# goofoo/SLR

Hardware: AMD Instinct MI355X
Metric: Msamples/sec @1024spp 1280x720 (unidirectional path tracing, Cornell_Box_Spheres-shaped scene) (higher is better)
Workload: dtype f32; 1 GPU; BASELINE configs[1]: Cornell_Box_Spheres walls/light/camera (TestScenes/Cornell_Box_Spheres.txt:8-107,132-138) + two tessellated spheres (aluminium mirror, Lambert), 4428 triangles, RGB mode, 1280x720, 1024 spp, seed 1509761209; stripes=0, tree=host binned SAH

## Files before the change

### slr_amd/csrc/pt_kernels.h

```cpp
#pragma once
#include <hip/hip_runtime.h>
#include <stdint.h>

#include "device_types.h"

namespace slrhip {

static const int kLdsMaterials = 32;
static const int kLdsLights = 16;
static const int kLdsSpectra = 96;
static const int kLdsPoolFloats = 6144;

struct DevScene {
    const float4* nodes;
    const float4* leafTris;
    const ShadeTri* shadeTris;
    const LightTri* lightTris;
    const DevMaterial* materials;
    const DevMaterialS* materialsS;
    const DevSpectrum* spectra;
    const float* spectrumPool;
    const float* lightPMF;
    const float* lightCDF;
    uint32_t numNodes;
// ... 51 lines not shown

struct PathBuffers {
    uint4* rng;
    float4* rayOrg;
    float4* rayDir;
    float4* hit;
    int32_t* hitInstance;
    float4* alpha;
    float4* spR;
    float4* spC;
    float4* results;
    float4* fbSum;
    float4* fbComp;
    float4* nee;
    float4* shadowDir;
    float* pdfPrev;
    uint4* hdr;
    uint32_t* flags;
    uint32_t* cursor;
    uint32_t* visible;
    uint32_t* shadowQueue;
    uint32_t* tailList;
    uint32_t* queueCount;
    uint32_t* activeSlots;
    uint32_t* idleShards;
    uint32_t* blockDead;
    uint32_t* errorWord;
    uint32_t* tailMode;
    uint32_t* tailWords;
    uint32_t* tailIdled;
    uint32_t* windowSamples;
    uint64_t* totals;
    const uint32_t* pixelXY;
    uint32_t rayStride, spStride, hdrStride;
};

struct RenderParams {
    uint32_t numSlots;
    uint32_t numBlocks;
    uint32_t numPixels, stripes;
    uint32_t sppBegin, sppCount;
    uint32_t workItems;
    uint32_t numWaves;
    uint32_t runLength;
    uint32_t numRuns;
    int32_t rngSeed;
    float timeStart, timeEnd;
    uint32_t imageWidth, imageHeight;
    uint32_t countSlots;
    uint32_t shardCapacity;
    uint32_t spectral;
    uint32_t injectError;
    uint32_t tailSlots;
};

static const uint32_t kWorkRotate = 40503u;
struct WorkItem {
    uint32_t pix, pass;
    bool valid;
};
__host__ __device__ inline uint32_t workRun(const RenderParams& rp, uint32_t wave, uint32_t j) {
    return j * rp.numWaves + (uint32_t)(((uint64_t)wave + (uint64_t)j * kWorkRotate) % rp.numWaves);
}
__host__ __device__ inline WorkItem workItemOf(const RenderParams& rp, uint32_t wave, uint32_t taken) {
    const uint32_t j = taken / rp.runLength, r = taken - j * rp.runLength;
    WorkItem w;
    w.pix = 0; w.pass = 0; w.valid = false;
    if (j > rp.numRuns / rp.numWaves) return w;
    const uint32_t run = workRun(rp, wave, j);
    if (run >= rp.numRuns) return w;
    const uint32_t group = run / rp.numPixels;
    w.pix = run - group * rp.numPixels;
    w.pass = group * rp.runLength + r;
    w.valid = true;
    return w;
}
__host__ __device__ inline uint32_t workSamplesTaken(const RenderParams& rp, uint32_t wave, uint32_t taken) {
    uint32_t runs = 0;
    for (uint32_t j = 0; j <= rp.numRuns / rp.numWaves; ++j) if (workRun(rp, wave, j) < rp.numRuns) ++runs;
    const uint32_t length = runs * rp.runLength;
    return taken < length ? taken : length;
}

__device__ __forceinline__ uint32_t liveSlots(const PathBuffers& pb, uint32_t numSlots) {
    uint32_t idle = 0;
#pragma unroll
    for (uint32_t k = 0; k < kShards; ++k) idle += pb.idleShards[k * kCounterStride];
    return numSlots - idle;
}
__device__ __forceinline__ bool tailModeBegins(const PathBuffers& pb, uint32_t live, uint32_t tailSlots, uint32_t parity) {
    if (tailSlots == 0u) return false;
    if (pb.tailMode[0]) return true;
    if (live > tailSlots) return false;
    if (blockIdx.x == 0 && threadIdx.x == 0) pb.tailMode[0] = 1u + parity;
    return true;
}

void launchResetSlots(const PathBuffers& pb, const RenderParams& rp, bool clearSensor, hipStream_t stream);
void launchFold(const PathBuffers& pb, const RenderParams& rp, hipStream_t stream);
void launchShade(const DevScene& sc, const PathBuffers& pb, const RenderParams& rp, uint32_t parity, hipStream_t stream);
void launchCountSamples(const PathBuffers& pb, const RenderParams& rp, hipStream_t stream);
void launchTail(const DevScene& sc, const PathBuffers& pb, const RenderParams& rp, uint32_t liveSlots, int numCUs, hipStream_t stream);
bool tailKernelAvailable(const DevScene& sc, bool spectral);
void launchResolve(const PathBuffers& pb, const RenderParams& rp, float* dst, hipStream_t stream);
void launchBsdfQueries(const DevScene& sc, bool spectral, uint32_t material, uint32_t n, const float* in, float wlOffset, uint32_t wl,
                       float4* geo, float4* misc, float4* fsSample, float4* fsEval, hipStream_t stream);
// ... 30 lines not shown
```

### slr_amd/csrc/pt_shade_kernels.h

```cpp
#pragma once
#include <hip/hip_runtime.h>
#include <stdlib.h>

#include <string>

#include "pt_bsdf.h"
#include "pt_bsdf_multi.h"
#include "pt_camera.h"
#include "pt_kernels.h"
#include "pt_surface.h"
#include "pt_tex.h"

namespace slrhip {

enum : uint32_t {
    ST_IDLE = 0,
    ST_REGEN = 1,
    ST_FIRST_HIT = 2,
    ST_NEXT_HIT = 3,
    ST_FINISH = 4
};
#define F_STATE(f) ((f) & 7u)
#define F_PATHLEN(f) (((f) >> 3) & 127u)
#define F_WL(f) (((f) >> 16) & 15u)
#define F_WLSEL(f) (((f) >> 12) & 1u)
#define F_DELTA(f) (((f) >> 13) & 1u)
#define F_SHADOW(f) (((f) >> 14) & 1u)
#define F_HASPATH(f) (((f) >> 15) & 1u)
#define F_SPVALID(f) (((f) >> 10) & 1u)
#define F_MAKE(state, len, wl, wlsel, delta, shadow) \
    ((state) | ((len) << 3) | ((wl) << 16) | ((wlsel) << 12) | ((delta) << 13) | ((shadow) << 14))

static const int kShadeBlock = 256;

template <class S> struct SpecIO;
template <> struct SpecIO<RGB> {
    static __device__ __forceinline__ void load(const float4* a, const float* , uint32_t slot, uint32_t , RGB& v, float& w) {
        const float4 q = a[slot];
        v = RGB(q.x, q.y, q.z); w = q.w;
    }
    static __device__ __forceinline__ void store(float4* a, float* , uint32_t slot, uint32_t , const RGB& v, float w) {
        a[slot] = make_float4(v.r, v.g, v.b, w);
    }
};
template <> struct SpecIO<Spec16> {
    static __device__ __forceinline__ void load(const float4* a, const float* scalars, uint32_t slot, uint32_t n, Spec16& v, float& w) {
#pragma unroll
        for (int p = 0; p < 4; ++p) {
            const float4 q = a[(size_t)p * n + slot];
            v.c[4 * p] = q.x; v.c[4 * p + 1] = q.y; v.c[4 * p + 2] = q.z; v.c[4 * p + 3] = q.w;
        }
        w = scalars ? scalars[slot] : 0.0f;
    }
    static __device__ __forceinline__ void store(float4* a, float* scalars, uint32_t slot, uint32_t n, const Spec16& v, float w) {
#pragma unroll
        for (int p = 0; p < 4; ++p) a[(size_t)p * n + slot] = make_float4(v.c[4 * p], v.c[4 * p + 1], v.c[4 * p + 2], v.c[4 * p + 3]);
        if (scalars) scalars[slot] = w;
    }
};

template <class S> struct MatIO;
template <> struct MatIO<RGB> {
    template <bool LDS>
    static __device__ __forceinline__ Mat<RGB> load(const DevScene& sc, const float4* ldsMats, uint32_t idx, float) {
// ... 251 lines not shown
    __device__ __forceinline__ void end(const PathBuffers&, uint32_t, uint32_t, bool) {}
};

template <bool SPECTRAL>
struct ShadeLds {
    float4 mats[SPECTRAL ? kLdsMaterials * 2 + kLdsSpectra * 2 + kLdsPoolFloats / 4 : kLdsMaterials * 5];
    float4 lights[kLdsLights * 9];
    float lightPMF[kLdsLights];
    float lightCDF[kLdsLights + 4];
};
static_assert(kLdsLights % 4 == 0, "the light PMF is staged as whole float4");

template <bool SPECTRAL>
__device__ __forceinline__ void stageShadeTables(const DevScene& sc, ShadeLds<SPECTRAL>& lds) {
    constexpr uint32_t kSegments = SPECTRAL ? 6u : 4u;
    constexpr uint32_t matsF4 = SPECTRAL ? kLdsMaterials * 2 + kLdsSpectra * 2 + kLdsPoolFloats / 4 : kLdsMaterials * 5;
    const uint32_t dst[6] = {0u,
                             SPECTRAL ? (uint32_t)(kLdsMaterials * 2) : matsF4,
                             SPECTRAL ? (uint32_t)(kLdsMaterials * 2 + kLdsSpectra * 2) : matsF4 + kLdsLights * 9,
                             SPECTRAL ? matsF4 : matsF4 + kLdsLights * 9 + kLdsLights / 4,
                             matsF4 + kLdsLights * 9,
                             matsF4 + kLdsLights * 9 + kLdsLights / 4};
    float4* out = reinterpret_cast<float4*>(&lds);
    const uint32_t total = sc.tableEnd[kSegments - 1];
    for (uint32_t base = threadIdx.x; base < total; base += 4 * kShadeBlock) {
        float4 v[4];
#pragma unroll
        for (int u = 0; u < 4; ++u) {
            const uint32_t i = base + u * kShadeBlock;
            v[u] = sc.shadeTables[min(i, total - 1u)];
        }
#pragma unroll
        for (int u = 0; u < 4; ++u) asm volatile("" : "+v"(v[u].x), "+v"(v[u].y), "+v"(v[u].z), "+v"(v[u].w));
#pragma unroll
        for (int u = 0; u < 4; ++u) {
            const uint32_t i = base + u * kShadeBlock;
            if (i >= total) continue;
            uint32_t begin = 0, to = dst[0];
#pragma unroll
            for (uint32_t k = 0; k + 1 < kSegments; ++k)
                if (i >= sc.tableEnd[k]) { begin = sc.tableEnd[k]; to = dst[k + 1]; }
            out[to + (i - begin)] = v[u];
        }
    }
}

#ifndef SLR_WAVES_SPECTRAL_GLOSSY
#define SLR_WAVES_SPECTRAL_GLOSSY 2
#endif
#ifndef SLR_WAVES_SPECTRAL
#define SLR_WAVES_SPECTRAL 3
#endif
#ifndef SLR_WAVES_RGB
#define SLR_WAVES_RGB 2
#endif
template <class S> struct TexSpectrum {
    static __device__ __forceinline__ S eval(const DevScene& sc, const DevTexture& t, float texU, float texV, float wlOffset) {
        if (t.kind == SLRHIP_TEXTURE_IMAGE_SPECTRUM) {
            const float* x = sc.texTexels + (size_t)imageTexel(t, texU, texV) * 3;
            const float kEqualEnergyReflectance = 0.009355121400914532f;
            return evaluateUpsampledRuntime<S>(sc, x[0], x[1], x[2] / kEqualEnergyReflectance, wlOffset);
        }
        return evalSpectrum<S>(sc.spectra, sc.spectrumPool, checkerIndex(t, texU, texV) ? t.spec1 : t.spec0, wlOffset);
    }
};
template <> struct TexSpectrum<RGB> {
    static __device__ __forceinline__ RGB eval(const DevScene& sc, const DevTexture& t, float texU, float texV, float) {
        if (t.kind == SLRHIP_TEXTURE_IMAGE_SPECTRUM) {
            const float* x = sc.texTexels + (size_t)imageTexel(t, texU, texV) * 3;
            return RGB(x[0], x[1], x[2]);
        }
        return checkerIndex(t, texU, texV) ? RGB(t.rgb1[0], t.rgb1[1], t.rgb1[2]) : RGB(t.rgb0[0], t.rgb0[1], t.rgb0[2]);
    }
};

template <class S>
__device__ __forceinline__ int32_t texturizeMat(const DevScene& sc, Mat<S>& mm, uint32_t matIndex, float texU, float texV, float wlOffset) {
    mm.type &= ~kMatTexturedBit;
    const int4 mt = *reinterpret_cast<const int4*>(sc.matTex + matIndex);
    if (mt.x >= 0) { const DevTexture t = loadTexture(sc.textures, (uint32_t)mt.x); mm.a = 1.0f * TexSpectrum<S>::eval(sc, t, texU, texV, wlOffset); }
    if (mt.y >= 0) { const DevTexture t = loadTexture(sc.textures, (uint32_t)mt.y); mm.b = TexSpectrum<S>::eval(sc, t, texU, texV, wlOffset); }
    if (mt.z >= 0) { const DevTexture t = loadTexture(sc.textures, (uint32_t)mt.z); mm.c = TexSpectrum<S>::eval(sc, t, texU, texV, wlOffset); }
    return mt.w;
}

template <class S>
struct SlotLoads {
    uint4 r4;
    S alpha;
    float pdfPrev;
    float4 h, o4, d4;
    int32_t hitInstance;
    float wlOffset;
    __device__ __forceinline__ void issue(const DevScene& sc, const PathBuffers& pb, const RenderParams& rp, uint32_t slot) {
        r4 = pb.rng[(size_t)slot * pb.hdrStride];
        SpecIO<S>::load(pb.alpha, pb.pdfPrev, slot, rp.numSlots, alpha, pdfPrev);
        h = pb.hit[slot];
        hitInstance = sc.instances ? pb.hitInstance[slot] : -1;
        o4 = pb.rayOrg[(size_t)slot * pb.rayStride];
        d4 = pb.rayDir[(size_t)slot * pb.rayStride];
        wlOffset = S::N == 3 ? 0.0f : __uint_as_float(pb.hdr[(size_t)slot * pb.hdrStride].z);
    }
};

template <class S, bool LDS_TABLES, bool MF, bool MULTI, bool TEX, bool FUSED>
__device__ __forceinline__ void logicSlot(const DevScene& sc, const PathBuffers& pb, const RenderParams& rp, const ShadeLds<S::N != 3>& lds,
                                          const float* lightPMF, const float* lightCDF, uint32_t slot, const SlotLoads<S>& in, uint32_t& flags, uint32_t vis,
// ... 265 lines not shown

        flags |= sp.validBits();
        if (FUSED && emitRegen) {
            radiance = sp.total();
        }
        else {
            pb.flags[slot] = flags;
            sp.end(pb, slot, rp.numSlots, !emitRegen);
        }
        if (!emitRegen) {
            pb.rng[(size_t)slot * pb.hdrStride] = make_uint4(rng.s0, rng.s1, rng.s2, rng.s3);
            SpecIO<S>::store(pb.alpha, pb.pdfPrev, slot, rp.numSlots, alpha, bsdfPDFprev);
        }
        if (emitExt) {
            pb.rayOrg[(size_t)slot * pb.rayStride] = make_float4(rayOrg.x, rayOrg.y, rayOrg.z, rayTmin);
            pb.rayDir[(size_t)slot * pb.rayStride] = make_float4(rayDir.x, rayDir.y, rayDir.z, INFINITY);
        }
    }
}

__device__ __forceinline__ RGB storageAddend(const RGB& val, float) { return val; }
__device__ __forceinline__ Spec16 storageAddend(const Spec16& val, float wlOffset) {
    const float recBinWidth = 16 / (830.0f - 360.0f);
    uint32_t sBin[16];
    float v[16];
    bool near = true;
#pragma unroll
    for (int i = 0; i < 16; ++i) {
        sBin[i] = min((uint32_t)((wavelengthOf(i, wlOffset) - 360.0f) / (830.0f - 360.0f) * 16), 15u);
        v[i] = val.c[i] * recBinWidth;
        near = near && (sBin[i] + 1u >= (uint32_t)i) && (sBin[i] <= (uint32_t)i + 1u);
    }
    Spec16 addend;
    if (near) {
#pragma unroll
        for (int b = 0; b < 16; ++b) {
            float a = 0.0f;
            if (b > 0) a = (sBin[b - 1] == (uint32_t)b) ? a + v[b - 1] : a;
            a = (sBin[b] == (uint32_t)b) ? a + v[b] : a;
            if (b < 15) a = (sBin[b + 1] == (uint32_t)b) ? a + v[b + 1] : a;
            addend.c[b] = a;
        }
    }
    else {
#pragma unroll
        for (int i = 0; i < 16; ++i) {
#pragma unroll
            for (int b = 0; b < 16; ++b) addend.c[b] = (sBin[i] == (uint32_t)b) ? addend.c[b] + v[i] : addend.c[b];
        }
    }
    return addend;
}

template <class S>
__device__ __forceinline__ void startSample(const DevScene& sc, const PathBuffers& pb, const RenderParams& rp, uint32_t slot, uint32_t pix,
                                            uint32_t passOfWindow) {
    const uint32_t xy = pb.pixelXY[pix];
    const uint32_t px = xy & 0xFFFFu, py = xy >> 16;
    Rng rng;
    const CameraDraws draws = drawCameraSample(rng, rp.rngSeed, px, py, rp.sppBegin + passOfWindow, rp.timeStart, rp.timeEnd);
    const float wlOffset = draws.wlOffset;
    const uint32_t wl = min((uint32_t)(uint16_t)(S::N * draws.uLambda), (uint32_t)(S::N - 1));
    const float selectWLPDF = S::N == 3 ? 1.0f : S::N / (830.0f - 360.0f);
    const CameraRay cam = sampleCameraRay(sc.camera, rp.imageWidth, rp.imageHeight, draws);
    const V3 lensP = cam.org, lensN = cam.lensN, rayDir = cam.dir;
    float dirPDF = sc.camera.imgPlaneDistance * sc.camera.imgPlaneDistance /
                   ((cam.dirLocalZ * cam.dirLocalZ * cam.dirLocalZ) * sc.camera.imgPlaneArea);
    float camWeight = absDot(rayDir, lensN) / (sc.camera.areaPDF * dirPDF * selectWLPDF);
    pb.flags[slot] = F_MAKE((uint32_t)ST_FIRST_HIT, 0u, wl, 0u, 0u, 0u);
    pb.rng[(size_t)slot * pb.hdrStride] = make_uint4(rng.s0, rng.s1, rng.s2, rng.s3);
    pb.hdr[(size_t)slot * pb.hdrStride] = make_uint4(pix, __float_as_uint(camWeight), __float_as_uint(wlOffset), passOfWindow);
    pb.rayOrg[(size_t)slot * pb.rayStride] = make_float4(lensP.x, lensP.y, lensP.z, 0.0f);
    pb.rayDir[(size_t)slot * pb.rayStride] = make_float4(rayDir.x, rayDir.y, rayDir.z, INFINITY);
}

__device__ __forceinline__ void storeResult(float4* results, size_t entry, const RGB& v) { results[entry] = make_float4(v.r, v.g, v.b, 0.0f); }
__device__ __forceinline__ void storeResult(float4* results, size_t entry, const Spec16& v) {
#pragma unroll
    for (int k = 0; k < 4; ++k) results[entry * 4 + k] = make_float4(v.c[4 * k], v.c[4 * k + 1], v.c[4 * k + 2], v.c[4 * k + 3]);
}
template <class S>
__device__ __forceinline__ void writeResult(const PathBuffers& pb, const RenderParams& rp, uint32_t slot, uint32_t flags, const uint4& hdr,
                                            bool inRegisters, S C) {
    float unusedW;
    const float camW = __uint_as_float(hdr.y);
    if (!inRegisters) {
        C = S();
        if (F_SPVALID(flags)) SpecIO<S>::load(pb.spR, nullptr, slot * pb.spStride, rp.numSlots * pb.spStride, C, unusedW);
    }
    const S weight = (S(1.0f) * S(1.0f)) * camW;
    storeResult(pb.results, (size_t)hdr.w * rp.numPixels + hdr.x, storageAddend(weight * C, S::N == 3 ? 0.0f : __uint_as_float(hdr.z)));
}

struct StartLds {
    uint32_t lane[kShadeBlock];
    uint32_t pix[kShadeBlock];
    uint32_t pass[kShadeBlock];
    uint32_t waveBase[kShadeBlock / 64 + 1];
    uint32_t wentIdle;
};

#ifndef SLR_SHADE_EARLY
#define SLR_SHADE_EARLY 1
#endif
template <class S, bool LDS_TABLES, bool MF, bool MULTI = false, bool TEX = false>
__global__ __launch_bounds__(kShadeBlock)
__attribute__((amdgpu_waves_per_eu(S::N == 3 ? SLR_WAVES_RGB : (MF ? SLR_WAVES_SPECTRAL_GLOSSY : SLR_WAVES_SPECTRAL)))) void k_shade(DevScene sc, PathBuffers pb, RenderParams rp, uint32_t parity) {
    __shared__ ShadeLds<S::N != 3> lds;
    __shared__ PushLds pushLds;
    __shared__ StartLds start;
    const uint32_t slot = blockIdx.x * kShadeBlock + threadIdx.x;
    const uint32_t lane = threadIdx.x & 63u, wave = threadIdx.x >> 6;

    {
        const uint32_t liveSlots = pb.activeSlots[0], tailMode = pb.tailMode[0], dead = pb.blockDead[blockIdx.x];
        if ((liveSlots == 0u) | (tailMode != 0u) | (dead != 0u)) return;
    }

    uint32_t flags = pb.flags[slot];
    const uint32_t vis = pb.visible[slot];
    SlotLoads<S> in;
    if (SLR_SHADE_EARLY) in.issue(sc, pb, rp, slot);
    const uint32_t state0 = F_STATE(flags);
    const uint32_t globalWave = blockIdx.x * (kShadeBlock / 64) + wave;
    const uint32_t taken = pb.cursor[globalWave];
    if (threadIdx.x == 0) start.wentIdle = 0u;
    if (LDS_TABLES) stageShadeTables<S::N != 3>(sc, lds);
    {
        const int anyWork = __syncthreads_or(state0 != ST_IDLE);
        if (!anyWork) {
            if (threadIdx.x == 0) pb.blockDead[blockIdx.x] = 1u;
            return;
        }
    }
    if (!SLR_SHADE_EARLY) in.issue(sc, pb, rp, slot);
    const float* lightPMF = LDS_TABLES ? lds.lightPMF : sc.lightPMF;
    const float* lightCDF = LDS_TABLES ? lds.lightCDF : sc.lightCDF;

    bool emitExt = false, emitShadow = false, pathEnded = false;
    S radiance;
    if (state0 == ST_FIRST_HIT || state0 == ST_NEXT_HIT || state0 == ST_FINISH)
        logicSlot<S, LDS_TABLES, MF, MULTI, TEX, true>(sc, pb, rp, lds, lightPMF, lightCDF, slot, in, flags, vis, radiance, emitExt, emitShadow, pathEnded);

    if (pathEnded) {
        const uint4 hdr = pb.hdr[(size_t)slot * pb.hdrStride];
        writeResult<S>(pb, rp, slot, flags, hdr, S::N == 3, radiance);
    }
    blockPush(pushLds, emitShadow, slot, pb.shadowQueue, pb.queueCount + parity * kQueueSetWords, rp.shardCapacity, pb.errorWord);
    if (rp.countSlots) {
        const uint64_t ma = __ballot(emitExt || emitShadow || pathEnded);
        if (lane == 0 && ma) atomicAdd((unsigned long long*)&pb.totals[totalIndex(T_SLOT_VISITS, blockIdx.x % kShards)], (unsigned long long)__popcll(ma));
    }

    const bool wants = pathEnded || state0 == ST_REGEN;
    {
        const uint64_t mw = __ballot(wants);
        WorkItem w;
        w.valid = false;
        if (wants) w = workItemOf(rp, globalWave, taken + (uint32_t)__popcll(mw & ((1ull << lane) - 1ull)));
        if (lane == 0 && mw) pb.cursor[globalWave] = taken + (uint32_t)__popcll(mw);
        const bool becameIdle = wants && !w.valid;
        if (becameIdle) pb.flags[slot] = F_MAKE((uint32_t)ST_IDLE, 0u, 0u, 0u, 0u, 0u);
        const uint64_t mi = __ballot(becameIdle);
        if (lane == 0 && mi) atomicAdd(&start.wentIdle, (uint32_t)__popcll(mi));
        const bool starts = wants && w.valid;
        const uint64_t ms = __ballot(starts);
        if (lane == 0) start.waveBase[wave] = (uint32_t)__popcll(ms);
        __syncthreads();
        uint32_t base = 0;
        for (uint32_t k = 0; k < wave; ++k) base += start.waveBase[k];
        if (starts) {
            const uint32_t i = base + (uint32_t)__popcll(ms & ((1ull << lane) - 1ull));
            start.lane[i] = threadIdx.x;
            start.pix[i] = w.pix;
            start.pass[i] = w.pass;
        }
        __syncthreads();
        if (threadIdx.x == 0 && start.wentIdle) atomicAdd(&pb.idleShards[(blockIdx.x % kShards) * kCounterStride], start.wentIdle);
        const uint32_t n = start.waveBase[0] + start.waveBase[1] + start.waveBase[2] + start.waveBase[3];
        if (threadIdx.x < n)
            startSample<S>(sc, pb, rp, blockIdx.x * kShadeBlock + start.lane[threadIdx.x], start.pix[threadIdx.x], start.pass[threadIdx.x]);
    }
}

template <class S>
__global__ void k_reset_slots(PathBuffers pb, RenderParams rp, uint32_t clearSensor) {
    const uint32_t slot = blockIdx.x * blockDim.x + threadIdx.x;
    pb.flags[slot] = F_MAKE((uint32_t)ST_REGEN, 0u, 0u, 0u, 0u, 0u);
    pb.hdr[(size_t)slot * pb.hdrStride] = make_uint4(0u, 0u, 0u, 0u);
    pb.visible[slot] = 0;
    if (threadIdx.x == 0) pb.blockDead[blockIdx.x] = 0u;
    if ((threadIdx.x & 63u) == 0u) pb.cursor[slot >> 6] = 0u;
    if (clearSensor) {
        constexpr uint32_t planes = S::N == 3 ? 1u : 4u;
        for (size_t e = slot; e < (size_t)rp.numPixels * planes; e += (size_t)gridDim.x * blockDim.x) {
            pb.fbSum[e] = make_float4(0.0f, 0.0f, 0.0f, 0.0f);
            pb.fbComp[e] = make_float4(0.0f, 0.0f, 0.0f, 0.0f);
        }
    }
    if (blockIdx.x == 0) {
        for (uint32_t k = threadIdx.x; k < 2 * kQueueSetWords; k += blockDim.x) pb.queueCount[k] = 0;
        if (threadIdx.x < kShards) pb.idleShards[threadIdx.x * kCounterStride] = 0u;
        if (threadIdx.x == 0) {
            pb.activeSlots[0] = rp.numSlots; pb.errorWord[0] = rp.injectError ? ERR_QUEUE_OVERFLOW : 0u;
            pb.tailMode[0] = 0u; pb.tailWords[0] = 0u; pb.tailWords[1] = 0u; pb.tailIdled[0] = 0u; pb.windowSamples[0] = 0u;
        }
    }
}

template <class S>
__global__ void k_resolve(PathBuffers pb, RenderParams rp, float* dst) {
    const uint32_t pix = blockIdx.x * blockDim.x + threadIdx.x;
    if (pix >= rp.numPixels) return;
    const uint32_t xy = pb.pixelXY[pix];
    const uint32_t px = xy & 0xFFFFu, py = xy >> 16;
    float* o = dst + ((size_t)py * rp.imageWidth + px) * S::N;
    if (S::N == 3) {
        const float4 v = pb.fbSum[pix];
        o[0] = v.x; o[1] = v.y; o[2] = v.z;
    }
    else {
#pragma unroll
        for (int k = 0; k < 4; ++k) {
            const float4 v = pb.fbSum[(size_t)pix * 4 + k];
            o[4 * k] = v.x; o[4 * k + 1] = v.y; o[4 * k + 2] = v.z; o[4 * k + 3] = v.w;
        }
    }
}

template <class S>
__global__ void __launch_bounds__(64) k_bsdf_queries(DevScene sc, uint32_t material, uint32_t n, const float* __restrict__ in, float wlOffset,
                                                     uint32_t wl, float4* __restrict__ geo, float4* __restrict__ misc,
                                                     float4* __restrict__ fsSample, float4* __restrict__ fsEval) {
    const uint32_t i = blockIdx.x * blockDim.x + threadIdx.x;
// ... 38 lines not shown
```

### slr_amd/csrc/slrhip_api.hip

```cpp
#include <hip/hip_runtime.h>
#include <dlfcn.h>

#include <algorithm>
#include <atomic>
#include <chrono>
#include <cmath>
#include <cstdio>
#include <cstring>
#include <string>
#include <vector>

#include "../../include/slrhip.h"
#include "bvh.h"
#include "pt_kernels.h"
#include "render_plan.h"
#include "scene_prep.h"

using namespace slrhip;

namespace {

const int kDefaultPairs = 1;
const uint32_t kStatusWords = 8;
enum StatusWord : uint32_t {
// ... 212 lines not shown
        if (const int rc = checkTreeLimits(g.depth, g.numNodes, g.numLeafTris,
                                           "device-built tree deeper than the 64-entry traversal stack (QBVH.h:299); use the host build", &err)) {
            for (void* a : {(void*)g.nodes, (void*)g.nodesQ, (void*)g.leafTris, (void*)g.shadeTris}) (void)hipFree(a);
            return fail(rc, err);
        }
        ctx->nodes.adopt(g.nodes, g.numNodes);
        ctx->leafTris.adopt(g.leafTris, g.numLeafTris);
        ctx->shadeTris.adopt(g.shadeTris, d.num_triangles);
        quantized = g.nodesQ != nullptr && useQuantizedNodes(g.numNodes);
        if (quantized) ctx->nodesQ.adopt(g.nodesQ, g.numNodes); else (void)hipFree(g.nodesQ);
        numNodes = g.numNodes; depth = g.depth; leafRefs = g.numLeafTris;
    }
    else {
        HIP_TRY(ctx->nodes.upload(p.bvh.nodes));
        if (p.quantized) HIP_TRY(ctx->nodesQ.upload(p.bvh.quantized));
        if (p.wide8) HIP_TRY(ctx->nodes8.upload(p.bvh.nodes8));
        HIP_TRY(ctx->leafTris.upload(p.bvh.leafTris));
    }
    HIP_TRY(ctx->textures.upload(p.textures));
    HIP_TRY(ctx->texTexels.upload(p.texTexels));
    HIP_TRY(ctx->matTex.upload(p.matTex));
    HIP_TRY(ctx->triUV.upload(p.triUV));
    HIP_TRY(ctx->alphaTris.upload(p.alphaTris));
    if (p.build != TreeBuild::Device) HIP_TRY(ctx->shadeTris.upload(p.shadeTris));
    HIP_TRY(ctx->lightTris.upload(p.lightTris));
    HIP_TRY(ctx->instances.upload(p.instances));
    HIP_TRY(ctx->materials.upload(p.materials));
    HIP_TRY(ctx->materialsS.upload(p.materialsS));
    HIP_TRY(ctx->spectrumPool.upload(p.spectrumPool));
    HIP_TRY(ctx->spectra.upload(p.spectra));
    HIP_TRY(ctx->lightPMF.upload(p.lightPMF));
    HIP_TRY(ctx->lightCDF.upload(p.lightCDF));
    HIP_TRY(ctx->shadeTables.upload(p.shadeTables));
    HIP_TRY(ctx->envTexels.upload(p.envTexels));
    HIP_TRY(ctx->envTopPDF.upload(p.envTopPDF)); HIP_TRY(ctx->envTopCDF.upload(p.envTopCDF));
    HIP_TRY(ctx->envRowPDF.upload(p.envRowPDF)); HIP_TRY(ctx->envRowCDF.upload(p.envRowCDF));
    HIP_TRY(ctx->gridCells.upload(p.gridCells)); HIP_TRY(ctx->pointUV.upload(p.pointUV)); HIP_TRY(ctx->pointSpectrum.upload(p.pointSpectrum));
    HIP_TRY(ctx->queryError.alloc(1));
    HIP_TRY(hipMemset(ctx->queryError.ptr, 0, sizeof(uint32_t)));
    bindScene(ctx, d, p, numNodes, quantized);
    ctx->bvhDepth = depth;
    ctx->bvhLeafRefs = leafRefs;
    ctx->haveScene = true;
    return SLRHIP_OK;
}

static long autoStripesOverride() { static const long v = [] { const char* e = tuningEnv("SLRHIP_AUTO_STRIPES"); return e ? atol(e) : 0L; }(); return v; }
static int pairsMask() { static const int v = [] { const char* e = tuningEnv("SLRHIP_PAIRS"); return e ? atoi(e) : kDefaultPairs; }(); return v; }
static uint32_t runLengthOverride() {
    static const uint32_t v = [] { const char* e = getenv("SLRHIP_RUN_LENGTH"); const long n = e ? atol(e) : 0L; return n >= 1 && n <= 4096 ? (uint32_t)n : 0u; }();
    return v;
}

static size_t frameFloats(const RenderParams& rp) { return (size_t)rp.imageWidth * rp.imageHeight * (rp.spectral ? 16 : 3); }

static void bindBuffers(slrhip_ctx* ctx, const FramePlan& plan) {
    PathBuffers pb{};
    pb.rayStride = plan.rayStride; pb.spStride = plan.spStride; pb.hdrStride = plan.hdrStride;
    pb.rayOrg = ctx->rayOrg.ptr; pb.rayDir = plan.rayStride == 2 ? ctx->rayOrg.ptr + 1 : ctx->rayDir.ptr;
    pb.spR = ctx->spR.ptr; pb.spC = plan.spStride == 2 ? ctx->spR.ptr + 1 : ctx->spC.ptr;
    pb.hdr = ctx->hdr.ptr; pb.rng = plan.hdrStride == 2 ? ctx->hdr.ptr + 1 : ctx->rng.ptr;
    pb.hit = ctx->hit.ptr; pb.hitInstance = ctx->scene.instances ? ctx->hitInstance.ptr : nullptr;
    pb.alpha = ctx->alpha.ptr; pb.pdfPrev = plan.spectral ? ctx->pdfPrev.ptr : nullptr;
    pb.nee = ctx->nee.ptr; pb.shadowDir = ctx->shadowDir.ptr; pb.visible = ctx->visible.ptr; pb.flags = ctx->flags.ptr;
    pb.results = ctx->results.ptr; pb.fbSum = ctx->fbSum.ptr; pb.fbComp = ctx->fbComp.ptr; pb.pixelXY = ctx->pixelXY.ptr;
    pb.cursor = ctx->cursor.ptr; pb.shadowQueue = ctx->shadowQueue.ptr; pb.tailList = ctx->tailList.ptr; pb.queueCount = ctx->queueCount.ptr;
    pb.idleShards = ctx->idleShards.ptr; pb.blockDead = ctx->blockDead.ptr; pb.totals = ctx->totals.ptr;
    uint32_t* const status = ctx->activeSlots.ptr;
    pb.activeSlots = status + S_LIVE; pb.errorWord = status + S_ERROR; pb.windowSamples = status + S_WINDOW_SAMPLES;
    pb.tailIdled = status + S_TAIL_IDLED; pb.tailMode = status + S_TAIL_MODE; pb.tailWords = status + S_TAIL_LENGTH;
    ctx->buffers = pb;
}

static hipError_t readStatus(slrhip_ctx* ctx, uint32_t* words, uint32_t count, hipStream_t s) {
    const hipError_t e = hipMemcpyAsync(words, ctx->activeSlots.ptr, count * sizeof(uint32_t), hipMemcpyDeviceToHost, s);
    return e == hipSuccess ? hipStreamSynchronize(s) : e;
}

static int checkWindow(slrhip_ctx* ctx, hipStream_t s) {
    uint32_t words[kStatusWords] = {};
    HIP_TRY(readStatus(ctx, words, kStatusWords, s));
    if (words[S_ERROR]) return deviceError(words[S_ERROR]);
    if (words[S_WINDOW_SAMPLES] != ctx->params.workItems)
        return fail(SLRHIP_ERR_HIP, "slrhip_render: the work queues handed out " + std::to_string(words[S_WINDOW_SAMPLES]) + " samples for a window of " +
                                        std::to_string(ctx->params.workItems) + " (internal error)");
    return SLRHIP_OK;
}

static int runTail(slrhip_ctx* ctx, uint32_t* status, hipStream_t s, bool timed) {
    struct Timer {
        hipEvent_t t0 = nullptr, t1 = nullptr;
        ~Timer() { if (t0) (void)hipEventDestroy(t0); if (t1) (void)hipEventDestroy(t1); }
    } timer;
    if (timed) { HIP_TRY(hipEventCreate(&timer.t0)); HIP_TRY(hipEventCreate(&timer.t1)); HIP_TRY(hipEventRecord(timer.t0, s)); }
    launchTail(ctx->scene, ctx->buffers, ctx->params, status[S_LIVE], ctx->numCUs, s);
    if (timed) HIP_TRY(hipEventRecord(timer.t1, s));
    HIP_TRY(hipGetLastError());
    const uint32_t liveBefore = status[S_LIVE];
    uint32_t words[S_TAIL_CURSOR + 1] = {};
    HIP_TRY(readStatus(ctx, words, S_TAIL_CURSOR + 1, s));
    std::memcpy(status, words, (S_TAIL_MODE + 1) * sizeof(uint32_t));
    if (timed) {
        float ms = 0.0f;
        HIP_TRY(hipEventElapsedTime(&ms, timer.t0, timer.t1));
        ctx->profMs[SLRHIP_KERNEL_TAIL] += ms;
        ++ctx->profLaunches[SLRHIP_KERNEL_TAIL];
// ... 166 lines not shown

int slrhip_upload_scene(slrhip_ctx* ctx, const slrhip_scene_desc* d) {
    if (!ctx || !d) return fail(SLRHIP_ERR_INVALID_ARGUMENT, "slrhip_upload_scene: null argument");
    const auto t0 = std::chrono::steady_clock::now();
    PreparedScene p;
    std::string err;
    if (const int rc = prepareScene(*d, ctx->config, &p, &err)) return fail(rc, err);
    if (const int rc = commitScene(ctx, *d, p)) return rc;
    ctx->buildSeconds = std::chrono::duration<double>(std::chrono::steady_clock::now() - t0).count();
    return SLRHIP_OK;
}

int slrhip_render_begin(slrhip_ctx* ctx, const slrhip_render_settings* st, slrhip_shard shard) {
    if (!ctx || !st) return fail(SLRHIP_ERR_INVALID_ARGUMENT, "slrhip_render_begin: null argument");
    if (!ctx->haveScene) return fail(SLRHIP_ERR_NO_SCENE, "slrhip_render_begin: no scene uploaded");
    const bool spectral = ctx->config.mode == SLRHIP_MODE_SPECTRAL;
    FramePlan plan;
    std::string err;
    if (const int rc = planFrame(st->image_width, st->image_height, shard.shard_index, shard.shard_count, ctx->config.stripes, spectral,
                                 autoStripesOverride(), pairsMask(), &plan, &err))
        return fail(rc, err);
    ctx->haveRender = false;
    HIP_TRY(hipSetDevice(ctx->device));
    const size_t slots = plan.slotCapacity, planes = spectral ? 4 : 1, pixels = std::max(plan.numPixels, 1u);
    hipError_t e = ctx->pixelXY.upload(shardPixels(plan));
    const auto alloc = [&e](auto& array, size_t n, bool skew) { if (e == hipSuccess) e = array.alloc(n, skew); };
    alloc(ctx->rayOrg, slots * plan.rayStride, true); alloc(ctx->rayDir, plan.rayStride == 2 ? 1 : slots, true); alloc(ctx->hit, slots, true);
    alloc(ctx->alpha, slots * planes, true); alloc(ctx->spR, slots * planes * plan.spStride, true); alloc(ctx->spC, plan.spStride == 2 ? 1 : slots * planes, true);
    alloc(ctx->fbSum, pixels * planes, true); alloc(ctx->fbComp, pixels * planes, true);
    alloc(ctx->nee, slots * planes, true); alloc(ctx->shadowDir, slots, true); alloc(ctx->pdfPrev, spectral ? slots : 1, true);
    alloc(ctx->hdr, slots * plan.hdrStride, true); alloc(ctx->rng, plan.hdrStride == 2 ? 1 : slots, true);
    alloc(ctx->cursor, slots / 64u, false); alloc(ctx->idleShards, kShards * kCounterStride, false);
    alloc(ctx->flags, slots, true); alloc(ctx->visible, slots, true);
    if (ctx->scene.instances) alloc(ctx->hitInstance, slots, true);
    alloc(ctx->shadowQueue, (size_t)plan.shardCapacity * kShards, true); alloc(ctx->tailList, slots, true);
    alloc(ctx->blockDead, plan.numBlocks, false); alloc(ctx->queueCount, 2 * kQueueSetWords, false);
    alloc(ctx->activeSlots, kStatusWords, false); alloc(ctx->totals, (size_t)T_KINDS * kShards * kTotalStride, false);
    if (e != hipSuccess) return fail(SLRHIP_ERR_HIP, std::string("slrhip_render_begin: allocating the path state: ") + hipGetErrorString(e));
    HIP_TRY(hipMemsetAsync(ctx->totals.ptr, 0, ctx->totals.count * sizeof(uint64_t), nullptr));
    HIP_TRY(hipMemsetAsync(ctx->activeSlots.ptr, 0, kStatusWords * sizeof(uint32_t), nullptr));
    HIP_TRY(hipStreamSynchronize(nullptr));

    bindBuffers(ctx, plan);
    RenderParams rp{};
    rp.numSlots = plan.numSlots; rp.numBlocks = rp.numSlots / 256u; rp.numWaves = rp.numSlots / 64u;
    rp.numPixels = plan.numPixels; rp.stripes = plan.stripes;
    rp.runLength = 1;
    rp.rngSeed = st->rng_seed; rp.timeStart = st->time_start; rp.timeEnd = st->time_end;
    rp.imageWidth = plan.width; rp.imageHeight = plan.height;
    rp.countSlots = (ctx->config.flags & SLRHIP_FLAG_COUNT_TRAVERSAL) ? 1u : 0u;
    rp.shardCapacity = plan.shardCapacity;
    rp.spectral = spectral ? 1u : 0u;
    rp.injectError = (ctx->config.flags & SLRHIP_FLAG_TEST_DEVICE_ERROR) ? 1u : 0u;
    ctx->params = rp;
    ctx->settings = *st;
    ctx->shard = shard;
    ctx->iterations = 0;
    ctx->firstRenderCall = true;
    ctx->featReady = false; ctx->featChannels = 0; ctx->featPassEnd = 0;
    ctx->haveRender = true;
    return SLRHIP_OK;
}

int slrhip_render(slrhip_ctx* ctx, uint32_t sppBegin, uint32_t sppCount, void* streamPtr) {
    if (!ctx) return fail(SLRHIP_ERR_INVALID_ARGUMENT, "slrhip_render: null context");
    if (!ctx->haveRender) return fail(SLRHIP_ERR_NO_SCENE, "slrhip_render: call slrhip_render_begin first");
    HIP_TRY(hipSetDevice(ctx->device));
    hipStream_t stream = (hipStream_t)streamPtr;
    const RenderParams& rp = ctx->params;
    if (rp.numSlots == 0) { ctx->firstRenderCall = false; return SLRHIP_OK; }
    uint64_t budget = 16ull << 30;
    if (const char* e = getenv("SLRHIP_RESULT_WINDOW_MB")) { const long mb = atol(e); if (mb > 0) budget = (uint64_t)mb << 20; }
    const uint32_t window = planWindows(rp.numPixels, rp.spectral != 0, sppCount, budget);
    HIP_TRY(ctx->results.alloc((size_t)window * rp.numPixels * (rp.spectral ? 4u : 1u)));
    ctx->buffers.results = ctx->results.ptr;
    if (sppCount == 0) return renderWindow(ctx, sppBegin, 0, stream);
    for (uint32_t done = 0; done < sppCount; done += window) {
        const int rc = renderWindow(ctx, sppBegin + done, std::min(window, sppCount - done), stream);
        if (rc != SLRHIP_OK) return rc;
    }
    return SLRHIP_OK;
}

int slrhip_resolve_framebuffer(slrhip_ctx* ctx, float* deviceDst, size_t numFloats, void* streamPtr) {
    if (!ctx || !deviceDst) return fail(SLRHIP_ERR_INVALID_ARGUMENT, "slrhip_resolve_framebuffer: null argument");
    if (!ctx->haveRender) return fail(SLRHIP_ERR_NO_SCENE, "slrhip_resolve_framebuffer: nothing rendered");
    const RenderParams& rp = ctx->params;
    const size_t need = frameFloats(rp);
    if (numFloats < need) return fail(SLRHIP_ERR_INVALID_ARGUMENT, "slrhip_resolve_framebuffer: destination too small");
    HIP_TRY(hipSetDevice(ctx->device));
    hipStream_t stream = (hipStream_t)streamPtr;
    HIP_TRY(hipMemsetAsync(deviceDst, 0, need * sizeof(float), stream));
    if (rp.numPixels) launchResolve(ctx->buffers, rp, deviceDst, stream);
    HIP_TRY(hipGetLastError());
    return SLRHIP_OK;
}

int slrhip_reduce_framebuffer(slrhip_ctx* ctx, void* ncclComm, int root, float* deviceDst, size_t numFloats, void* streamPtr) {
    if (!ctx || !ncclComm) return fail(SLRHIP_ERR_INVALID_ARGUMENT, "slrhip_reduce_framebuffer: null argument");
    if (!ctx->haveRender) return fail(SLRHIP_ERR_NO_SCENE, "slrhip_reduce_framebuffer: nothing rendered");
    const RenderParams& rp = ctx->params;
    const size_t need = frameFloats(rp);
    if (deviceDst && numFloats < need) return fail(SLRHIP_ERR_INVALID_ARGUMENT, "slrhip_reduce_framebuffer: destination too small");
    typedef int (*reduce_fn)(const void*, void*, size_t, int, int, int, void*, hipStream_t);
    typedef int (*rank_fn)(void*, int*);
    static void* rccl = [] {
        void* h = dlopen("librccl.so", RTLD_NOW | RTLD_GLOBAL);
        return h ? h : dlopen("librccl.so.1", RTLD_NOW | RTLD_GLOBAL);
    }();
    static reduce_fn ncclReduceFn = rccl ? reinterpret_cast<reduce_fn>(dlsym(rccl, "ncclReduce")) : nullptr;
    static rank_fn ncclCommUserRankFn = rccl ? reinterpret_cast<rank_fn>(dlsym(rccl, "ncclCommUserRank")) : nullptr;
    if (!ncclReduceFn || !ncclCommUserRankFn) return fail(SLRHIP_ERR_UNSUPPORTED, "slrhip_reduce_framebuffer: librccl.so (ncclReduce) not found");
    int myRank = -1;
    if (ncclCommUserRankFn(ncclComm, &myRank) != 0) return fail(SLRHIP_ERR_HIP, "slrhip_reduce_framebuffer: ncclCommUserRank failed");
    if (myRank == root && !deviceDst) return fail(SLRHIP_ERR_INVALID_ARGUMENT, "slrhip_reduce_framebuffer: the root rank needs a destination buffer");
    HIP_TRY(hipSetDevice(ctx->device));
    HIP_TRY(ctx->resolveScratch.alloc(need));
    int rc = slrhip_resolve_framebuffer(ctx, ctx->resolveScratch.ptr, need, streamPtr);
    if (rc != SLRHIP_OK) return rc;
    const int kNcclFloat32 = 7, kNcclSum = 0;
    const int nrc = ncclReduceFn(ctx->resolveScratch.ptr, deviceDst, need, kNcclFloat32, kNcclSum, root, ncclComm, (hipStream_t)streamPtr);
    if (nrc != 0) return fail(SLRHIP_ERR_HIP, "slrhip_reduce_framebuffer: ncclReduce failed (" + std::to_string(nrc) + ")");
    return SLRHIP_OK;
}

// ... 335 lines not shown
```

Before: 3034 Msamples/s.

## Fuse primary ray trace into shade kernel; raise RGB waves-per-EU hint

Adds an optional path, gated by the SLRHIP_PRIMARY env var, in which the shade kernel generates a new camera sample, traces the primary ray in place using an LDS traversal stack, and shades its first hit in the same launch. This skips the round trip of writing the ray state and running a separate trace pass. The path is off by default. Separately, the RGB waves_per_eu occupancy hint rises from 2 to 4, with a new glossy variant at 3, and this applies to every run. The result-window env parse now accepts fractional MB.

```diff
diff --git a/slr_amd/csrc/pt_kernels.h b/slr_amd/csrc/pt_kernels.h
--- a/slr_amd/csrc/pt_kernels.h
+++ b/slr_amd/csrc/pt_kernels.h
@@ -127,6 +127,7 @@
     uint32_t spectral;
     uint32_t injectError;
     uint32_t tailSlots;
+    uint32_t fusePrimary;
 };
 
 static const uint32_t kWorkRotate = 40503u;
diff --git a/slr_amd/csrc/pt_shade_kernels.h b/slr_amd/csrc/pt_shade_kernels.h
--- a/slr_amd/csrc/pt_shade_kernels.h
+++ b/slr_amd/csrc/pt_shade_kernels.h
@@ -10,6 +10,7 @@
 #include "pt_kernels.h"
 #include "pt_surface.h"
 #include "pt_tex.h"
+#include "pt_traverse.h"
 
 namespace slrhip {
 
@@ -367,7 +368,10 @@
 #define SLR_WAVES_SPECTRAL 3
 #endif
 #ifndef SLR_WAVES_RGB
-#define SLR_WAVES_RGB 2
+#define SLR_WAVES_RGB 4
+#endif
+#ifndef SLR_WAVES_RGB_GLOSSY
+#define SLR_WAVES_RGB_GLOSSY 3
 #endif
 template <class S> struct TexSpectrum {
     static __device__ __forceinline__ S eval(const DevScene& sc, const DevTexture& t, float texU, float texV, float wlOffset) {
@@ -739,9 +743,14 @@
     return addend;
 }
 
+struct SampleStart {
+    uint4 rng;
+    uint4 hdr;
+    float4 org, dir;
+    uint32_t flags;
+};
 template <class S>
-__device__ __forceinline__ void startSample(const DevScene& sc, const PathBuffers& pb, const RenderParams& rp, uint32_t slot, uint32_t pix,
-                                            uint32_t passOfWindow) {
+__device__ __forceinline__ SampleStart drawSample(const DevScene& sc, const PathBuffers& pb, const RenderParams& rp, uint32_t pix, uint32_t passOfWindow) {
     const uint32_t xy = pb.pixelXY[pix];
     const uint32_t px = xy & 0xFFFFu, py = xy >> 16;
     Rng rng;
@@ -754,11 +763,23 @@
     float dirPDF = sc.camera.imgPlaneDistance * sc.camera.imgPlaneDistance /
                    ((cam.dirLocalZ * cam.dirLocalZ * cam.dirLocalZ) * sc.camera.imgPlaneArea);
     float camWeight = absDot(rayDir, lensN) / (sc.camera.areaPDF * dirPDF * selectWLPDF);
-    pb.flags[slot] = F_MAKE((uint32_t)ST_FIRST_HIT, 0u, wl, 0u, 0u, 0u);
-    pb.rng[(size_t)slot * pb.hdrStride] = make_uint4(rng.s0, rng.s1, rng.s2, rng.s3);
-    pb.hdr[(size_t)slot * pb.hdrStride] = make_uint4(pix, __float_as_uint(camWeight), __float_as_uint(wlOffset), passOfWindow);
-    pb.rayOrg[(size_t)slot * pb.rayStride] = make_float4(lensP.x, lensP.y, lensP.z, 0.0f);
-    pb.rayDir[(size_t)slot * pb.rayStride] = make_float4(rayDir.x, rayDir.y, rayDir.z, INFINITY);
+    SampleStart s;
+    s.flags = F_MAKE((uint32_t)ST_FIRST_HIT, 0u, wl, 0u, 0u, 0u);
+    s.rng = make_uint4(rng.s0, rng.s1, rng.s2, rng.s3);
+    s.hdr = make_uint4(pix, __float_as_uint(camWeight), __float_as_uint(wlOffset), passOfWindow);
+    s.org = make_float4(lensP.x, lensP.y, lensP.z, 0.0f);
+    s.dir = make_float4(rayDir.x, rayDir.y, rayDir.z, INFINITY);
+    return s;
+}
+template <class S>
+__device__ __forceinline__ void startSample(const DevScene& sc, const PathBuffers& pb, const RenderParams& rp, uint32_t slot, uint32_t pix,
+                                            uint32_t passOfWindow) {
+    const SampleStart s = drawSample<S>(sc, pb, rp, pix, passOfWindow);
+    pb.flags[slot] = s.flags;
+    pb.rng[(size_t)slot * pb.hdrStride] = s.rng;
+    pb.hdr[(size_t)slot * pb.hdrStride] = s.hdr;
+    pb.rayOrg[(size_t)slot * pb.rayStride] = s.org;
+    pb.rayDir[(size_t)slot * pb.rayStride] = s.dir;
 }
 
 __device__ __forceinline__ void storeResult(float4* results, size_t entry, const RGB& v) { results[entry] = make_float4(v.r, v.g, v.b, 0.0f); }
@@ -785,6 +806,7 @@
     uint32_t pass[kShadeBlock];
     uint32_t waveBase[kShadeBlock / 64 + 1];
     uint32_t wentIdle;
+    uint32_t nodes, tris;
 };
 
 #ifndef SLR_SHADE_EARLY
@@ -792,10 +814,12 @@
 #endif
 template <class S, bool LDS_TABLES, bool MF, bool MULTI = false, bool TEX = false>
 __global__ __launch_bounds__(kShadeBlock)
-__attribute__((amdgpu_waves_per_eu(S::N == 3 ? SLR_WAVES_RGB : (MF ? SLR_WAVES_SPECTRAL_GLOSSY : SLR_WAVES_SPECTRAL)))) void k_shade(DevScene sc, PathBuffers pb, RenderParams rp, uint32_t parity) {
+__attribute__((amdgpu_waves_per_eu(S::N == 3 ? (MF ? SLR_WAVES_RGB_GLOSSY : SLR_WAVES_RGB) : (MF ? SLR_WAVES_SPECTRAL_GLOSSY : SLR_WAVES_SPECTRAL)))) void k_shade(DevScene sc, PathBuffers pb, RenderParams rp, uint32_t parity) {
     __shared__ ShadeLds<S::N != 3> lds;
     __shared__ PushLds pushLds;
     __shared__ StartLds start;
+    __shared__ uint32_t primaryStack[kLdsStack * kTraceBlock];
+    static_assert(kTraceBlock == kShadeBlock, "traverse<> strides its LDS stack by kTraceBlock");
     const uint32_t slot = blockIdx.x * kShadeBlock + threadIdx.x;
     const uint32_t lane = threadIdx.x & 63u, wave = threadIdx.x >> 6;
 
@@ -805,13 +829,13 @@
     }
 
     uint32_t flags = pb.flags[slot];
-    const uint32_t vis = pb.visible[slot];
+    const uint32_t vis0 = pb.visible[slot];
     SlotLoads<S> in;
     if (SLR_SHADE_EARLY) in.issue(sc, pb, rp, slot);
     const uint32_t state0 = F_STATE(flags);
     const uint32_t globalWave = blockIdx.x * (kShadeBlock / 64) + wave;
     const uint32_t taken = pb.cursor[globalWave];
-    if (threadIdx.x == 0) start.wentIdle = 0u;
+    if (threadIdx.x == 0) { start.wentIdle = 0u; start.nodes = 0u; start.tris = 0u; }
     if (LDS_TABLES) stageShadeTables<S::N != 3>(sc, lds);
     {
         const int anyWork = __syncthreads_or(state0 != ST_IDLE);
@@ -824,23 +848,30 @@
     const float* lightPMF = LDS_TABLES ? lds.lightPMF : sc.lightPMF;
     const float* lightCDF = LDS_TABLES ? lds.lightCDF : sc.lightCDF;
 
-    bool emitExt = false, emitShadow = false, pathEnded = false;
-    S radiance;
-    if (state0 == ST_FIRST_HIT || state0 == ST_NEXT_HIT || state0 == ST_FINISH)
-        logicSlot<S, LDS_TABLES, MF, MULTI, TEX, true>(sc, pb, rp, lds, lightPMF, lightCDF, slot, in, flags, vis, radiance, emitExt, emitShadow, pathEnded);
-
-    if (pathEnded) {
-        const uint4 hdr = pb.hdr[(size_t)slot * pb.hdrStride];
-        writeResult<S>(pb, rp, slot, flags, hdr, S::N == 3, radiance);
-    }
-    blockPush(pushLds, emitShadow, slot, pb.shadowQueue, pb.queueCount + parity * kQueueSetWords, rp.shardCapacity, pb.errorWord);
-    if (rp.countSlots) {
-        const uint64_t ma = __ballot(emitExt || emitShadow || pathEnded);
-        if (lane == 0 && ma) atomicAdd((unsigned long long*)&pb.totals[totalIndex(T_SLOT_VISITS, blockIdx.x % kShards)], (unsigned long long)__popcll(ma));
-    }
-
-    const bool wants = pathEnded || state0 == ST_REGEN;
+    uint32_t visitSlot = slot, state = state0, vis = vis0;
+    uint4 hdr = make_uint4(0u, 0u, 0u, 0u);
+    bool pathEnded = false;
+    const auto visit = [&](const bool second) {
+        bool emitExt = false, emitShadow = false;
+        pathEnded = false;
+        S radiance;
+        if (state == ST_FIRST_HIT || state == ST_NEXT_HIT || state == ST_FINISH)
+            logicSlot<S, LDS_TABLES, MF, MULTI, TEX, true>(sc, pb, rp, lds, lightPMF, lightCDF, visitSlot, in, flags, vis, radiance, emitExt, emitShadow, pathEnded);
+
+        if (pathEnded) {
+            if (!second) hdr = pb.hdr[(size_t)visitSlot * pb.hdrStride];
+            writeResult<S>(pb, rp, visitSlot, flags, hdr, S::N == 3, radiance);
+            if (second) pb.flags[visitSlot] = F_MAKE((uint32_t)ST_REGEN, 0u, 0u, 0u, 0u, 0u);
+        }
+        blockPush(pushLds, emitShadow, visitSlot, pb.shadowQueue, pb.queueCount + parity * kQueueSetWords, rp.shardCapacity, pb.errorWord);
+        if (rp.countSlots) {
+            const uint64_t ma = __ballot(emitExt || emitShadow || pathEnded);
+            if (lane == 0 && ma) atomicAdd((unsigned long long*)&pb.totals[totalIndex(T_SLOT_VISITS, blockIdx.x % kShards)], (unsigned long long)__popcll(ma));
+        }
+    };
+    visit(false);
     {
+        const bool wants = pathEnded || state0 == ST_REGEN;
         const uint64_t mw = __ballot(wants);
         WorkItem w;
         w.valid = false;
@@ -865,8 +896,46 @@
         __syncthreads();
         if (threadIdx.x == 0 && start.wentIdle) atomicAdd(&pb.idleShards[(blockIdx.x % kShards) * kCounterStride], start.wentIdle);
         const uint32_t n = start.waveBase[0] + start.waveBase[1] + start.waveBase[2] + start.waveBase[3];
-        if (threadIdx.x < n)
-            startSample<S>(sc, pb, rp, blockIdx.x * kShadeBlock + start.lane[threadIdx.x], start.pix[threadIdx.x], start.pass[threadIdx.x]);
+        if (!rp.fusePrimary) {
+            if (threadIdx.x < n)
+                startSample<S>(sc, pb, rp, blockIdx.x * kShadeBlock + start.lane[threadIdx.x], start.pix[threadIdx.x], start.pass[threadIdx.x]);
+            return;
+        }
+        if (n == 0) return;
+
+        if (threadIdx.x == 0) atomicAdd((unsigned long long*)&pb.totals[totalIndex(T_EXT_RAYS, blockIdx.x % kShards)], (unsigned long long)n);
+        state = ST_IDLE;
+        TravCount cnt = {0, 0};
+        if (threadIdx.x < n) {
+            visitSlot = blockIdx.x * kShadeBlock + start.lane[threadIdx.x];
+            const SampleStart s = drawSample<S>(sc, pb, rp, start.pix[threadIdx.x], start.pass[threadIdx.x]);
+            hdr = s.hdr;
+            pb.hdr[(size_t)visitSlot * pb.hdrStride] = hdr;
+            HitRec hit;
+            uint32_t* const stack = primaryStack + threadIdx.x;
+            const V3 org(s.org.x, s.org.y, s.org.z), dir(s.dir.x, s.dir.y, s.dir.z);
+            if (sc.instances) traverse<false, true, true>(sc, sc.nodes, sc.leafTris, nullptr, 0u, org, dir, s.org.w, s.dir.w, &hit, stack, &cnt, pb.errorWord);
+            else traverse<false, true, false>(sc, sc.nodes, sc.leafTris, nullptr, 0u, org, dir, s.org.w, s.dir.w, &hit, stack, &cnt, pb.errorWord);
+            in.r4 = s.rng;
+            in.h = make_float4(__uint_as_float(hit.tri), hit.t, hit.b1, hit.b2);
+            in.hitInstance = sc.instances ? hit.inst : -1;
+            in.o4 = s.org; in.d4 = s.dir;
+            in.wlOffset = S::N == 3 ? 0.0f : __uint_as_float(hdr.z);
+            flags = s.flags;
+            vis = 0u;
+            state = ST_FIRST_HIT;
+        }
+        if (rp.countSlots) {
+            uint32_t nodes = cnt.nodes, tris = cnt.tris;
+            for (int off = 32; off > 0; off >>= 1) { nodes += __shfl_down(nodes, off); tris += __shfl_down(tris, off); }
+            if (lane == 0 && nodes) atomicAdd(&start.nodes, nodes);
+            if (lane == 0 && tris) atomicAdd(&start.tris, tris);
+        }
+    }
+    visit(true);
+    if (rp.countSlots && threadIdx.x == 0) {
+        if (start.nodes) atomicAdd((unsigned long long*)&pb.totals[totalIndex(T_NODES_CLOSEST, blockIdx.x % kShards)], (unsigned long long)start.nodes);
+        if (start.tris) atomicAdd((unsigned long long*)&pb.totals[totalIndex(T_TRIS_CLOSEST, blockIdx.x % kShards)], (unsigned long long)start.tris);
     }
 }
 
diff --git a/slr_amd/csrc/slrhip_api.hip b/slr_amd/csrc/slrhip_api.hip
--- a/slr_amd/csrc/slrhip_api.hip
+++ b/slr_amd/csrc/slrhip_api.hip
@@ -288,6 +288,11 @@
     return v;
 }
 
+static int primaryOverride() {
+    static const int v = [] { const char* e = getenv("SLRHIP_PRIMARY"); return e && (e[0] == '0' || e[0] == '1') && e[1] == 0 ? e[0] - '0' : -1; }();
+    return v;
+}
+
 static size_t frameFloats(const RenderParams& rp) { return (size_t)rp.imageWidth * rp.imageHeight * (rp.spectral ? 16 : 3); }
 
 static void bindBuffers(slrhip_ctx* ctx, const FramePlan& plan) {
@@ -560,6 +565,7 @@
     rp.shardCapacity = plan.shardCapacity;
     rp.spectral = spectral ? 1u : 0u;
     rp.injectError = (ctx->config.flags & SLRHIP_FLAG_TEST_DEVICE_ERROR) ? 1u : 0u;
+    rp.fusePrimary = primaryOverride() == 1 ? 1u : 0u;
     ctx->params = rp;
     ctx->settings = *st;
     ctx->shard = shard;
@@ -578,7 +584,7 @@
     const RenderParams& rp = ctx->params;
     if (rp.numSlots == 0) { ctx->firstRenderCall = false; return SLRHIP_OK; }
     uint64_t budget = 16ull << 30;
-    if (const char* e = getenv("SLRHIP_RESULT_WINDOW_MB")) { const long mb = atol(e); if (mb > 0) budget = (uint64_t)mb << 20; }
+    if (const char* e = getenv("SLRHIP_RESULT_WINDOW_MB")) { const double mb = atof(e); if (mb > 0.0 && mb < 1e12) budget = (uint64_t)(mb * 1048576.0); }
     const uint32_t window = planWindows(rp.numPixels, rp.spectral != 0, sppCount, budget);
     HIP_TRY(ctx->results.alloc((size_t)window * rp.numPixels * (rp.spectral ? 4u : 1u)));
     ctx->buffers.results = ctx->results.ptr;
```

Result: no change. 3009 Msamples/s (-0.8%).
